# skipperro/selkies-gstreamer

Measured on AMD Instinct MI355X. Metric: encoded fps + glass-to-glass p50 ms at 1920x1080; concurrent 60fps sessions/node, higher is better.
Workload: dtype uint8 pixels / int32 integer transforms (bit-exact vs CPU reference); 1 GPU; model=H.264 Constrained Baseline CAVLC, striped stripes 64px, CRF 25, global_batch=8, seq_len=1, parallelism=session-parallel dp1 x 8 sessions/GPU, resolution=1920x1080, backend=hip, deblock=auto, me_full=True, upload_overlap=False, frames_in_flight=1, num_refs=1, numa_node_rank0=0

## Files before the change

### csrc/kernels/h264_gpu.h

```cpp
#pragma once
#include <hip/hip_runtime.h>
#include "../codec/overlay.h"
#include "../codec/h264_encoder.h"
#include "../codec/h264_frame.h"
#include "../codec/h264_deblock.h"

namespace sk {
namespace h264 {
namespace gpu {

constexpr int kMbSlotBytes = 1024;
constexpr int kSliceHdrMax = 64;
constexpr int kPackMaxSliceMbs = 16384;

struct Planes {
    uint8_t* y;
    uint8_t* u;
    uint8_t* v;
};

struct FrameArgs {
    int W, H, mb_w, mb_h, stride_y, stride_c, num_slices, rows_per_slice, fullframe;
    int full_range, me_range, me_iters;
    const uint8_t* bgrx;
// ... 6 lines not shown
    int* stripe_dirty;
    StripeState* plan_state;
    int* plan_ctl;
    const int* key_seq_host;
    int* key_dev;
    PlanConfig plan_cfg;
    SliceTask* tasks;
    MeResult* me;
    int16_t* mvfield;
    MbInfo* mbs;
    int16_t* coefs;
    uint32_t* mb_bits;
    int* mb_nbits;
    int* slice_info;
    int out_slot_bytes;
    const uint8_t* param_sets;
    const int* param_set_len;
    int param_set_stride;
    uint8_t* host_out;
    int* host_size;
    int* frame_params_dev;
    const int* frame_params_host;
    SliceTask* tasks_host;
    unsigned long long* dbg;
    const CavlcTables* cavlc_tabs;
    int num_refs;
    int deblock;
    int me_full;
    int aq_strength;
    int subpel;
    int intra4x4;
    const uint8_t* ov_img[kOverlaySlots];
    const OverlayParams* ov;
    int8_t* aq;
    DbInfo* db;
    uint4* dbe;
    int16_t* fs_mv;
    RcState* rc;
    long long* rc_slice;
    float rc_fps;
    int* rc_redo;
    int nal_per_slice;
    const int* gate;
    const uint8_t* yuv;
    int yuv_fmt;
    ltr::LtrConfig ltr_cfg;
    Planes ltr;
    size_t ltr_ny, ltr_nc;
    ltr::LtrState* ltr_state;
    ltr::LtrTask* ltr_task;
    uint32_t* ltr_part;
    uint32_t* ltr_sad;
    int* ltr_cnt;
};

#if defined(__HIPCC__)
__device__ __forceinline__ Planes ref0_planes(const FrameArgs& a, int s) {
    if (a.ltr_cfg.mode == ltr::LTR_SECOND_REF) return a.ref;
    const int j = __builtin_amdgcn_readfirstlane(a.ltr_task[s].slot);
    if (j < 0) return a.ref;
    return Planes{a.ltr.y + (size_t)j * a.ltr_ny, a.ltr.u + (size_t)j * a.ltr_nc, a.ltr.v + (size_t)j * a.ltr_nc};
}
#endif

void launch_convert_damage(const FrameArgs& a, hipStream_t s);
void launch_encode(const FrameArgs& a, hipStream_t s, bool guard = false);
void launch_frontend(const FrameArgs& a, hipStream_t s);
void launch_commit(const FrameArgs& a, hipStream_t s, bool filter = true, bool account = false);
void launch_rc_account(const FrameArgs& a, const int* sizes, int n, int stride, int per_slice, hipStream_t s);
void launch_rc_guard_sizes(const FrameArgs& a, const int* sizes, int n, int* redo, bool chained, hipStream_t s);

}
}
}
```

### csrc/kernels/h264_kernels.hip

```cpp
#include "h264_gpu.h"
#include "../codec/color.h"
#include "../codec/h264_mb.h"
#include "../codec/h264_ep.h"

namespace sk {
namespace h264 {
namespace gpu {

__device__ __forceinline__ int lane_id() { return threadIdx.x & 63; }

__device__ __forceinline__ void wave_sync() {
    __builtin_amdgcn_fence(__ATOMIC_RELEASE, "wavefront");
    __builtin_amdgcn_wave_barrier();
    __builtin_amdgcn_fence(__ATOMIC_ACQUIRE, "wavefront");
}

__device__ __forceinline__ int wave_sum(int v) {
    v += __builtin_amdgcn_mov_dpp(v, 0xB1, 0xF, 0xF, false);
    v += __builtin_amdgcn_mov_dpp(v, 0x4E, 0xF, 0xF, false);
    v += __builtin_amdgcn_mov_dpp(v, 0x124, 0xF, 0xF, false);
    v += __builtin_amdgcn_mov_dpp(v, 0x128, 0xF, 0xF, false);
    return __builtin_amdgcn_readlane(v, 0) + __builtin_amdgcn_readlane(v, 16) +
           __builtin_amdgcn_readlane(v, 32) + __builtin_amdgcn_readlane(v, 48);
}

__device__ __forceinline__ Planes ref1_planes(const FrameArgs& a, int s) {
    if (!a.ltr_cfg.slots) return a.ref1;
    const size_t j = (size_t)sk_max(a.ltr_task[s].slot, 0);
    return Planes{a.ltr.y + j * a.ltr_ny, a.ltr.u + j * a.ltr_nc, a.ltr.v + j * a.ltr_nc};
}

__device__ __forceinline__ bool split_i(const FrameArgs& a, const SliceTask& t) {
    return a.nal_per_slice > 1 && intra_split(t, a.mb_w, a.deblock, a.intra4x4);
}
__device__ __forceinline__ int slice_nals(const FrameArgs& a, const SliceTask& t) {
    if (t.final_action == ACT_NONE) return 0;
    return split_i(a, t) ? intra_sub_count(t.num_rows * a.mb_w) : 1;
}

__device__ __forceinline__ int wave_incl_scan_max(int v) {
    int l = threadIdx.x & 63;
#pragma unroll
    for (int o = 1; o < 64; o <<= 1) {
        int t = __shfl_up(v, o);
        if (l >= o) v = max(v, t);
    }
    return v;
}

__device__ __forceinline__ int wave_incl_scan(int v) {
    int l = lane_id();
#pragma unroll
    for (int o = 1; o < 64; o <<= 1) {
        int t = __shfl_up(v, o);
        if (l >= o) v += t;
    }
    return v;
}

__device__ __forceinline__ void load_cavlc_tables(CavlcTables& dst, const CavlcTables* src) {
    static_assert(sizeof(CavlcTables) % 4 == 0, "dword copy");
    const uint32_t* s = reinterpret_cast<const uint32_t*>(src);
    uint32_t* d = reinterpret_cast<uint32_t*>(&dst);
    for (int i = threadIdx.x; i < (int)(sizeof(CavlcTables) / 4); i += blockDim.x) d[i] = s[i];
}

template <int NW>
// ... 1770 lines not shown
    for (;;) {
        const int bound = cbp == 0 ? 96 : quant_bound(m.q, false, S, T, dbg, kCodeStampRow);
        if (qp + 6 > cap || bound <= mb_bit_budget(false)) break;
        qp += 6;
        wave_sync();
        cbp = quant_analyse(m.wl, m.wc, qp, false, S, m.sl, m.sc, m.q, dbg, kCodeStampRow);
    }
    STAMP_S(dbg, kCodeStampRow, 4);
    MbInfo mb;
    memset(&mb, 0, sizeof(mb));
    mb.type = MB_P_16x16;
    mb.cbp = (uint8_t)cbp;
    mb.qp = (uint8_t)qp;
    int rec_l[4], rec_c[4];
    uint32_t* g32 = reinterpret_cast<uint32_t*>(a.coefs + (size_t)idx * kCoefPerMb);
    if (cbp == 0) {
#pragma unroll
        for (int j = 0; j < 4; j++) {
            rec_l[j] = m.pred_l[j];
            rec_c[j] = m.pred_c[j];
        }
        for (int i = l; i < kCoefPerMb / 2; i += 64) g32[i] = 0;
    } else {
        recon_mb_lanes(qp, false, cbp, S, m.pred_l, m.pred_c, rec_l, rec_c, m.sl, m.sc);
        STAMP_S(dbg, kCodeStampRow, 5);
        const uint32_t* s32 = reinterpret_cast<const uint32_t*>(S.coef);
        for (int i = l; i < kCoefPerMb / 2; i += 64) g32[i] = s32[i];
    }
    STAMP_S(dbg, kCodeStampRow, 6);
    const int mvx = m.mvx, mvy = m.mvy, refi = m.refi, pmx = m.pmx, pmy = m.pmy, smx = m.smx, smy = m.smy;
    uint32_t rw = (uint32_t)rec_l[0] | ((uint32_t)rec_l[1] << 8) | ((uint32_t)rec_l[2] << 16) |
                  ((uint32_t)rec_l[3] << 24);
    *reinterpret_cast<uint32_t*>(a.rec.y + (size_t)py * a.stride_y + px) = rw;
    if (l < 32) {
        uint8_t* cr = comp ? a.rec.v : a.rec.u;
        uint32_t cw = (uint32_t)rec_c[0] | ((uint32_t)rec_c[1] << 8) | ((uint32_t)rec_c[2] << 16) |
                      ((uint32_t)rec_c[3] << 24);
        *reinterpret_cast<uint32_t*>(cr + (size_t)cy0 * a.stride_c + cx0) = cw;
    }
    STAMP_S(dbg, kCodeStampRow, 7);
    if (l == 0) {
        mb.mvx = (int16_t)mvx;
        mb.mvy = (int16_t)mvy;
        mb.ref = (uint8_t)refi;
        if (mb.cbp == 0 && refi == 0 && mvx == smx && mvy == smy) {
            mb.type = MB_P_SKIP;
        } else {
            mb.mvdx = (int16_t)(mvx - pmx);
            mb.mvdy = (int16_t)(mvy - pmy);
        }
        if (mb.cbp)
            for (int i = 0; i < 24; i++) mb.nnz[i] = S.nnz[i];
        a.mbs[idx] = mb;
    }
    STAMP_S(dbg, kCodeStampRow, 8);
}

__device__ __forceinline__ void intra_modes_wave(const int* src_l, const int* src_c, const uint8_t* topp, const uint8_t* leftp,
                                 int tl, const uint8_t* const* ctop, const uint8_t* const* cleft, const int* ctl,
                                 bool aT, bool aL, int* cdcp, int* luma_mode, int* chroma_mode,
                                 int* luma_sad = nullptr) {
    const int l = lane_id();
    const int b = l >> 2, r = l & 3;
    const int cl = l & 31, comp = cl >> 4, cb = (cl >> 2) & 3;
    const int lx = blk_x(b) * 4, ly = blk_y(b) * 4 + r;
    int dc = i16_dc(topp, leftp, aT, aL);
    int pa = 0, pb = 0, pc = 0;
    if (aT && aL) i16_plane_params(topp, leftp, tl, &pa, &pb, &pc);
    const int order[4] = {2, 0, 1, 3};
    int best_mode = 2, best_sad = 0x7fffffff;
    for (int oi = 0; oi < 4; oi++) {
        int m = order[oi];
        if ((m == 0 && !aT) || (m == 1 && !aL) || (m == 3 && !(aT && aL))) continue;
        int sad = 0;
#pragma unroll
        for (int j = 0; j < 4; j++)
            sad += sk_abs(src_l[j] - i16_pred_pixel(m, lx + j, ly, topp, leftp, tl, aT, aL, dc, pa, pb, pc));
        sad = wave_sum(sad);
        if (sad < best_sad) { best_sad = sad; best_mode = m; }
    }
    const uint8_t* ct = ctop[comp];
    const uint8_t* cf = cleft[comp];
    const int clx = (cb & 1) * 4, cly = (cb >> 1) * 4 + r;
    int qa = 0, qb = 0, qc = 0;
    if (aT && aL) chroma_plane_params(ct, cf, ctl[comp], &qa, &qb, &qc);
    if (l < 8) cdcp[l] = chroma_dc_block(l & 1, (l >> 1) & 1, ctop[l >> 2], cleft[l >> 2], aT, aL);
    wave_sync();
    const int cdc_mine = cdcp[comp * 4 + cb];
    int best_cm = 0, best_csad = 0x7fffffff;
    for (int m = 0; m < 4; m++) {
        if ((m == 1 && !aL) || (m == 2 && !aT) || (m == 3 && !(aT && aL))) continue;
        int sad = 0;
#pragma unroll
        for (int j = 0; j < 4; j++) {
            int x = clx + j, y = cly, v;
            if (m == 0) v = cdc_mine;
            else if (m == 1) v = cf[y];
            else if (m == 2) v = ct[x];
            else v = sk_clip255((qa + qb * (x - 3) + qc * (y - 3) + 16) >> 5);
            sad += sk_abs(src_c[j] - v);
        }
        sad = wave_sum(l < 32 ? sad : 0);
        if (sad < best_csad) { best_csad = sad; best_cm = m; }
    }
    *luma_mode = best_mode;
    *chroma_mode = best_cm;
// ... 139 lines not shown
            sad = quad_sum(sad);
            if (r == 0) sads[q * 9 + m] = i4_mode_ok(m, ref.hasT, ref.hasL) ? sad : -1;
        }
        wave_sync();
        const int lam = i4_lambda(t.qp);
        int total = 0;
        uint64_t modes = 0;
        for (int b = 0; b < 16; b++) {
            const int bx = blk_x(b), by = blk_y(b);
            const int ma = bx > 0 ? (int)((modes >> (4 * blk_from_xy(bx - 1, by))) & 15) : (aL ? 2 : -1);
            const int mt = by > 0 ? (int)((modes >> (4 * blk_from_xy(bx, by - 1))) & 15) : (aT ? 2 : -1);
            const int pm = i4_predicted(ma, mt);
            int best = 0x7fffffff, bm = I4_DC;
            for (int m = 0; m < 9; m++) {
                const int sd = sads[b * 9 + m];
                if (sd < 0) continue;
                const int cost = sd + lam * (m == pm ? 1 : 4);
                if (cost < best) { best = cost; bm = m; }
            }
            modes |= (uint64_t)bm << (4 * b);
            total += best;
        }
        cand.i4lo = (uint32_t)modes;
        cand.i4hi = (uint32_t)(modes >> 32);
        i4 = i4_wins(total, sad16, t.qp);
        wave_sync();
    }
    MbInfo mb;
    memset(&mb, 0, sizeof(mb));
    int qp;
    if (i4) {
        mb.type = MB_I4x4;
        mb.chroma_mode = (uint8_t)cmode;
        mb.i4lo = cand.i4lo;
        mb.i4hi = cand.i4hi;
        int rec_l[4], rec_c[4];
        qp = code_mb_i4(src_smp, src_l, src_c, pred_c, start >= 0 ? start : t.qp, t.qp, aT, aL, aTR, S, mb, rec_l,
                        rec_c, nullptr, T);
    } else {
        int rec_l[4], rec_c[4];
        qp = code_mb(src_l, pred_l, src_c, pred_c, t.qp, true, S, mb, rec_l, rec_c, nullptr, T, nullptr, 0, start,
                     true);
    }
    if (l == 0) {
        MbInfo o;
        memset(&o, 0, sizeof(o));
        o.type = i4 ? MB_I4x4 : MB_I16x16;
        o.i16_mode = (uint8_t)mode;
        o.chroma_mode = (uint8_t)cmode;
        o.qp = (uint8_t)qp;
        o.i4lo = cand.i4lo;
        o.i4hi = cand.i4hi;
        a.mbs[idx] = o;
    }
}

__global__ __launch_bounds__(256) void k_code_inter(FrameArgs a) {
    if (a.gate && *a.gate == 0) return;
    __shared__ MbScratch Sw[4];
    __shared__ QpelLds Qw[4];
    __shared__ CavlcTables T;
    const int w = threadIdx.x >> 6;
    const int nmb = a.mb_w * a.mb_h;
    const int idx = xcd_remap(blockIdx.x, gridDim.x) * 4 + w;
    const bool valid = idx < nmb;
    const int mbx = valid ? idx % a.mb_w : 0, mby = valid ? idx / a.mb_w : 0;
    const int s = mby / a.rows_per_slice;
    const SliceTask t = a.tasks[s];
    if (valid && t.final_action == ACT_SKIPALL && lane_id() == 0) {
        MbInfo z;
        memset(&z, 0, sizeof(z));
        a.mbs[idx] = z;
        a.me[idx].mvx = 0;
        a.me[idx].mvy = 0;
        a.me[idx].ref = 0;
        a.me[idx].fx = a.me[idx].fy = 0;
    }
    const bool is_p = valid && t.final_action == ACT_P, is_i = valid && t.final_action == ACT_I;
    constexpr int kTabWords = (int)(sizeof(CavlcTables) / 4);
    static_assert(kTabWords <= 512, "two dwords per thread");
    const uint32_t* tab_src = reinterpret_cast<const uint32_t*>(a.cavlc_tabs);
    const uint32_t tab0 = tab_src[threadIdx.x];
    const uint32_t tab1 = threadIdx.x + 256 < kTabWords ? tab_src[threadIdx.x + 256] : 0u;
    InterMb m;
    bool need_tables = is_i;
    if (is_p) need_tables = code_inter_begin(a, t, s, idx, mbx, mby, Sw[w], Qw[w], m) != 0;
    if (__syncthreads_or(need_tables)) {
        uint32_t* tab_dst = reinterpret_cast<uint32_t*>(&T);
        tab_dst[threadIdx.x] = tab0;
        if (threadIdx.x + 256 < kTabWords) tab_dst[threadIdx.x + 256] = tab1;
        __syncthreads();
    }
    static_assert(sizeof(QpelLds) >= 64, "the pre-pass keeps its neighbour samples in the wave's QpelLds");
    if (is_p) code_inter_finish(a, t, idx, mbx, mby, Sw[w], T, m);
    else if (is_i) intra_prep_wave(a, t, idx, mbx, mby, Sw[w], reinterpret_cast<uint8_t*>(&Qw[w]), T);
}

constexpr int kMaxRows = 16;
struct IntraEdges {
    uint8_t bot_y[kMaxRows][4][16];
    uint8_t bot_c[kMaxRows][4][2][8];
    uint8_t right_y[kMaxRows][16];
    uint8_t right_c[kMaxRows][2][8];
};

struct IntraSrc {
    uint32_t y[64];
    uint32_t c[32];
    int mode, cmode, qp, i4;
    uint32_t i4m[2];
};
constexpr int kIntraRing = 4;

template <int MAXROWS>
__global__ __launch_bounds__(64 * (MAXROWS + 1)) void k_code_intra(FrameArgs a) {
    if (a.gate && *a.gate == 0) return;
    __shared__ MbScratch Sw[MAXROWS];
    __shared__ IntraEdges E;
    __shared__ IntraSrc R[MAXROWS][kIntraRing];
    __shared__ uint8_t zero16[16];
    __shared__ CavlcTables T;
    int s = blockIdx.x;
    const SliceTask t = a.tasks[s];
    if (t.final_action != ACT_I || split_i(a, t)) return;
#ifdef SK_STAMPS
// ... 87 lines not shown
                const bool is_i4 = __builtin_amdgcn_readfirstlane(in.i4) != 0;
                int pred_l[4], pred_c[4];
                intra_pred_lanes(is_i4 ? 2 : mode, cmode, nb, tl, ctl, aT, aL, pred_l, pred_c);
                STAMP(step, 2);
                MbInfo mb;
                memset(&mb, 0, sizeof(mb));
                mb.chroma_mode = (uint8_t)cmode;
                int rec_l[4], rec_c[4];
                if (is_i4) {
                    const bool aTR = aT && mbx + 1 < a.mb_w;
                    if (l < 4) S.nbtr[l] = aTR ? E.bot_y[w - 1][(mbx + 1) & 3][l] : 0;
                    const uint32_t m0 = __builtin_amdgcn_readfirstlane(in.i4m[0]);
                    const uint32_t m1 = __builtin_amdgcn_readfirstlane(in.i4m[1]);
                    mb.i4lo = m0;
                    mb.i4hi = m1;
                    mb.type = MB_I4x4;
                    wave_sync();
                    auto smp = [&](int x, int y) __attribute__((always_inline)) -> int {
                        if (y >= 0 && x >= 0) return S.ry[y * 16 + x];
                        if (y < 0) return x < 0 ? tl : (x < 16 ? (int)nb[x] : (int)S.nbtr[x - 16]);
                        return nb[16 + y];
                    };
                    code_mb_i4(smp, src_l, src_c, pred_c, start_qp, t.qp, aT, aL, aTR, S, mb, rec_l, rec_c,
                               a.coefs + (size_t)idx * kCoefPerMb, T);
                } else {
                    mb.type = MB_I16x16;
                    mb.i16_mode = (uint8_t)mode;
                    code_mb(src_l, pred_l, src_c, pred_c, t.qp, true, S, mb, rec_l, rec_c,
                            a.coefs + (size_t)idx * kCoefPerMb, T, a.dbg, step, start_qp);
                }
                STAMP(step, 6);
                wave_sync();
                if (ly == 15)
                    for (int j = 0; j < 4; j++) E.bot_y[w][mbx & 3][lx + j] = (uint8_t)rec_l[j];
                if (lx + 3 == 15) E.right_y[w][ly] = (uint8_t)rec_l[3];
                if (l < 32) {
                    if (cly == 7)
                        for (int j = 0; j < 4; j++) E.bot_c[w][mbx & 3][comp][clx + j] = (uint8_t)rec_c[j];
                    if (clx + 3 == 7) E.right_c[w][comp][cly] = (uint8_t)rec_c[3];
                }
                const int px = mbx * 16 + lx, py = mby * 16 + ly;
                uint32_t rw = (uint32_t)rec_l[0] | ((uint32_t)rec_l[1] << 8) | ((uint32_t)rec_l[2] << 16) |
                              ((uint32_t)rec_l[3] << 24);
                *reinterpret_cast<uint32_t*>(a.rec.y + (size_t)py * a.stride_y + px) = rw;
                if (l < 32) {
                    uint8_t* crp = comp ? a.rec.v : a.rec.u;
                    uint32_t cw = (uint32_t)rec_c[0] | ((uint32_t)rec_c[1] << 8) | ((uint32_t)rec_c[2] << 16) |
                                  ((uint32_t)rec_c[3] << 24);
                    *reinterpret_cast<uint32_t*>(crp + (size_t)(mby * 8 + cly) * a.stride_c + mbx * 8 + clx) = cw;
                }
                if (l == 0) {
                    for (int i = 0; i < 24; i++) mb.nnz[i] = S.nnz[i];
                    a.mbs[idx] = mb;
                    a.me[idx].mvx = 0;
                    a.me[idx].mvy = 0;
                    a.me[idx].ref = 0;
                    a.me[idx].fx = a.me[idx].fy = 0;
                }
                STAMP(step, 7);
            }
        }
        __syncthreads();
        if (w == 0) STAMP(step, 8);
    }
#ifdef SK_STAMPS
    if (a.dbg && threadIdx.x == 0 && blockIdx.x < 32) {
        a.dbg[1024 + 2 * blockIdx.x] = t_start;
        a.dbg[1024 + 2 * blockIdx.x + 1] = __builtin_amdgcn_s_memrealtime();
        if (blockIdx.x < 32) a.dbg[1024 + 64 + 2 * blockIdx.x] = __builtin_amdgcn_s_memtime() - c_start;
        if (blockIdx.x == SK_STAMP_BLOCK) {
            a.dbg[1024 + 200] = c_start;
            a.dbg[1024 + 201] = __builtin_amdgcn_s_memtime();
            a.dbg[1024 + 202] = c_loop;
            a.dbg[1024 + 203] = steps;
        }
        if (blockIdx.x < 32) a.dbg[1024 + 64 + 2 * blockIdx.x + 1] = __builtin_amdgcn_s_getreg((31 << 11) | 4);
    }
#endif
}

__global__ __launch_bounds__(256) void k_code_intra_sub(FrameArgs a) {
    if (a.gate && *a.gate == 0) return;
    __shared__ MbScratch Sw[4];
    __shared__ uint8_t right_y[4][16];
    __shared__ uint8_t right_c[4][2][8];
    __shared__ CavlcTables T;
    const int w = threadIdx.x >> 6, l = lane_id();
    const int gw = blockIdx.x * 4 + w;
    const int s = gw / a.nal_per_slice, j = gw % a.nal_per_slice;
    bool mine = false;
    SliceTask t;
    if (s < a.num_slices) {
        t = a.tasks[s];
        mine = split_i(a, t) && j < intra_sub_count(t.num_rows * a.mb_w);
    }
    if (!__syncthreads_or(mine)) return;
    load_cavlc_tables(T, a.cavlc_tabs);
    __syncthreads();
    if (!mine) return;
    MbScratch& S = Sw[w];
    const int b = l >> 2, r = l & 3;
    const int cl = l & 31, comp = cl >> 4, cb = (cl >> 2) & 3;
    const int lx = blk_x(b) * 4, ly = blk_y(b) * 4 + r;
    const int clx = (cb & 1) * 4, cly = (cb >> 1) * 4 + r;
    const int first = t.first_row * a.mb_w;
    const int k0 = j * kIntraSubMbs, k1 = sk_min(t.num_rows * a.mb_w, k0 + kIntraSubMbs);
// ... 19 lines not shown
        const uint32_t m1 = (uint32_t)__builtin_amdgcn_readfirstlane((int)pre.i4hi);
        int src_l[4], src_c[4];
#pragma unroll
        for (int q = 0; q < 4; q++) {
            src_l[q] = (sw >> (8 * q)) & 255;
            src_c[q] = (csw >> (8 * q)) & 255;
        }
        if (k + 1 < k1) fetch(k + 1, sw, csw, pre);
        uint8_t* nb = S.nb;
        {
            int v = 0;
            if (l >= 16 && l < 32) v = aL ? right_y[w][l - 16] : 0;
            else if (l >= 48) v = aL ? right_c[w][(l >> 3) & 1][l & 7] : 0;
            nb[l] = (uint8_t)v;
        }
        wave_sync();
        int pred_l[4], pred_c[4];
        intra_pred_lanes(is_i4 ? 2 : mode, cmode, nb, 0, zc, false, aL, pred_l, pred_c);
        MbInfo mb;
        memset(&mb, 0, sizeof(mb));
        mb.chroma_mode = (uint8_t)cmode;
        int rec_l[4], rec_c[4];
        if (is_i4) {
            mb.type = MB_I4x4;
            mb.i4lo = m0;
            mb.i4hi = m1;
            auto smp = [&](int x, int y) __attribute__((always_inline)) -> int {
                if (y >= 0 && x >= 0) return S.ry[y * 16 + x];
                if (y < 0) return 0;
                return nb[16 + y];
            };
            code_mb_i4(smp, src_l, src_c, pred_c, start_qp, t.qp, false, aL, false, S, mb, rec_l, rec_c,
                       a.coefs + (size_t)idx * kCoefPerMb, T);
        } else {
            mb.type = MB_I16x16;
            mb.i16_mode = (uint8_t)mode;
            code_mb(src_l, pred_l, src_c, pred_c, t.qp, true, S, mb, rec_l, rec_c, a.coefs + (size_t)idx * kCoefPerMb,
                    T, nullptr, 0, start_qp);
        }
        wave_sync();
        if (lx + 3 == 15) right_y[w][ly] = (uint8_t)rec_l[3];
        if (l < 32 && clx + 3 == 7) right_c[w][comp][cly] = (uint8_t)rec_c[3];
        const int px = mbx * 16 + lx, py = mby * 16 + ly;
        *reinterpret_cast<uint32_t*>(a.rec.y + (size_t)py * a.stride_y + px) =
            (uint32_t)rec_l[0] | ((uint32_t)rec_l[1] << 8) | ((uint32_t)rec_l[2] << 16) | ((uint32_t)rec_l[3] << 24);
        if (l < 32) {
            uint8_t* crp = comp ? a.rec.v : a.rec.u;
            *reinterpret_cast<uint32_t*>(crp + (size_t)(mby * 8 + cly) * a.stride_c + mbx * 8 + clx) =
                (uint32_t)rec_c[0] | ((uint32_t)rec_c[1] << 8) | ((uint32_t)rec_c[2] << 16) | ((uint32_t)rec_c[3] << 24);
        }
        if (l == 0) {
            for (int i = 0; i < 24; i++) mb.nnz[i] = S.nnz[i];
            a.mbs[idx] = mb;
            a.me[idx].mvx = 0;
            a.me[idx].mvy = 0;
            a.me[idx].ref = 0;
            a.me[idx].fx = a.me[idx].fy = 0;
        }
        wave_sync();
    }
}

constexpr int kCavlcStageWords = 24;
__global__ __launch_bounds__(256) void k_cavlc(FrameArgs a) {
    if (a.gate && *a.gate == 0) return;
    __shared__ uint32_t bits_w[4][kMbSlotBytes / 4];
    __shared__ uint32_t stage_w[4][27 * kCavlcStageWords];
    __shared__ int16_t coef_w[4][kCoefPerMb];
    __shared__ MbInfo mb_w[4];
    __shared__ CavlcTables T;
    load_cavlc_tables(T, a.cavlc_tabs);
    __syncthreads();
    uint32_t* bits = bits_w[threadIdx.x >> 6];
    int16_t* coef = coef_w[threadIdx.x >> 6];
    int nmb = a.mb_w * a.mb_h;
    int idx = xcd_remap(blockIdx.x, gridDim.x) * 4 + (threadIdx.x >> 6);
    if (idx >= nmb) return;
    int mbx = idx % a.mb_w, mby = idx / a.mb_w;
    int s = mby / a.rows_per_slice;
    const SliceTask t = a.tasks[s];
    if (t.final_action != ACT_P && t.final_action != ACT_I) return;
    int l = lane_id();
    MbInfo& mb = mb_w[threadIdx.x >> 6];
    if (l < (int)(sizeof(MbInfo) / 4))
        reinterpret_cast<uint32_t*>(&mb)[l] = reinterpret_cast<const uint32_t*>(a.mbs + idx)[l];
    wave_sync();
    if (mb.type == MB_P_SKIP) {
        if (l == 0) a.mb_nbits[idx] = 0;
        return;
    }
    bool p_slice = t.final_action == ACT_P;
    int first = t.first_row * a.mb_w;
    if (split_i(a, t)) first += ((idx - first) / kIntraSubMbs) * kIntraSubMbs;
    int run = 0;
    if (p_slice) {
        int j = idx - 1;
        while (j >= first) {
            int base = j - 63;
            int m = base + l;
            bool coded = m >= first && a.mbs[m].type != MB_P_SKIP;
            unsigned long long msk = __ballot(coded);
            if (msk) {
                int hi = 63 - __clzll(msk);
                run += j - (base + hi);
                break;
            }
            run += j - sk_max(base, first) + 1;
            j = base - 1;
        }
    }
    int qp_prev = t.qp;
    {
        int j = idx - 1;
        while (j >= first) {
            int base = j - 63;
            int m = base + l;
            bool has = m >= first && mb_has_qp_delta(a.mbs[m]);
            unsigned long long msk = __ballot(has);
            if (msk) {
                int hi = 63 - __clzll(msk);
                qp_prev = a.mbs[base + hi].qp;
                break;
            }
            j = base - 1;
        }
    }
    for (int i = l; i < kMbSlotBytes / 4; i += 64) bits[i] = 0;
    uint32_t* stage_all = stage_w[threadIdx.x >> 6];
    for (int i = l; i < 27 * kCavlcStageWords; i += 64) stage_all[i] = 0;
    const int16_t* gc = a.coefs + (size_t)idx * kCoefPerMb;
    for (int i = l; i < kCoefPerMb / 2; i += 64)
        reinterpret_cast<uint32_t*>(coef)[i] = reinterpret_cast<const uint32_t*>(gc)[i];
    wave_sync();
    MbNeighbours nb;
    nb.left = mbx > 0 && idx - 1 >= first ? &a.mbs[idx - 1] : nullptr;
    nb.top = mby > t.first_row && idx - a.mb_w >= first ? &a.mbs[idx - a.mb_w] : nullptr;
    int hdr_bits = 0;
    if (l == 0) {
        AtomicBitWriter w{bits, 0};
        if (p_slice) put_ue(w, (uint32_t)run);
        int dq = mb_has_qp_delta(mb) ? (int)mb.qp - qp_prev : 0;
        write_mb_header(w, mb, p_slice, dq, p_slice ? t.num_refs : 1, nb);
        hdr_bits = (int)w.pos;
    }
    hdr_bits = __shfl(hdr_bits, 0);
    int cbp_l = mb.cbp & 15, cbp_c = (mb.cbp >> 4) & 3;
    bool i16 = mb.type == MB_I16x16;
    const int16_t* bc = nullptr;
    int maxn = 0, nc = 0;
    bool act = false;
    if (l == 0) {
        if (i16) { act = true; bc = coef + kCoefLumaDC; maxn = 16; nc = luma_nc(mb, nb, 0); }
    } else if (l <= 16) {
        int blk = l - 1;
        if (i16) {
            if (cbp_l) { act = true; bc = coef + kCoefLuma + blk * 16 + 1; maxn = 15; }
        } else if (cbp_l & (1 << (blk >> 2))) {
            act = true; bc = coef + kCoefLuma + blk * 16; maxn = 16;
        }
        if (act) nc = luma_nc(mb, nb, blk);
    } else if (l <= 18) {
        if (cbp_c) { act = true; bc = coef + kCoefChromaDC + (l - 17) * 4; maxn = 4; nc = -1; }
    } else if (l <= 26) {
        if (cbp_c == 2) {
            int k = l - 19, c = k >> 2, bb = k & 3;
            act = true; bc = coef + kCoefChromaAC + (c * 4 + bb) * 16 + 1; maxn = 15;
            nc = chroma_nc(mb, nb, c, bb);
        }
    }
    int nbits = 0;
    uint32_t* stage = stage_all + (l < 27 ? l : 0) * kCavlcStageWords;
    StageBitWriter sw{stage, 0, kCavlcStageWords * 32, false};
    if (act) {
        cavlc_block(sw, bc, maxn, nc, T);
        nbits = (int)sw.pos;
    }
    int incl = wave_incl_scan(nbits);
    int off = hdr_bits + incl - nbits;
    if (act) {
        if (!sw.ovf) {
            const uint32_t sh = (uint32_t)off & 31;
            uint32_t wi = (uint32_t)off >> 5;
            for (int k = 0; k < (nbits + 31) >> 5; k++, wi++) {
                const uint32_t v = stage[k];
                atomicOr(&bits[wi], v >> sh);
                const uint32_t lo = sh ? v << (32 - sh) : 0u;
                if (lo) atomicOr(&bits[wi + 1], lo);
            }
        } else {
// ... 307 lines not shown
    const int nmbs = sk_min(16, a.mb_w - mbx0);
    if (tid < nmbs) {
        const int idx = mby * a.mb_w + mbx0 + tid;
        const bool zero = fin == ACT_SKIPALL;
        a.mvfield[2 * idx] = zero ? 0 : a.me[idx].mvx;
        a.mvfield[2 * idx + 1] = zero ? 0 : a.me[idx].mvy;
    }
    auto copy = [&](const Planes& src, const Planes& dst) {
        {
            const int row = tid >> 4, v = tid & 15;
            if (v < nmbs) {
                const size_t o = (size_t)(mby * 16 + row) * a.stride_y + (mbx0 + v) * 16;
                *reinterpret_cast<uint4*>(dst.y + o) = *reinterpret_cast<const uint4*>(src.y + o);
            }
        }
        if (tid < 128) {
            const int comp = tid >> 6, row = (tid >> 3) & 7, v = tid & 7;
            if (2 * v < nmbs) {
                const size_t o = (size_t)(mby * 8 + row) * a.stride_c + (mbx0 + 2 * v) * 8;
                uint8_t* d = comp ? dst.v : dst.u;
                const uint8_t* sp = comp ? src.v : src.u;
                if (2 * v + 1 < nmbs && (a.stride_c & 15) == 0) {
                    *reinterpret_cast<uint4*>(d + o) = *reinterpret_cast<const uint4*>(sp + o);
                } else {
                    *reinterpret_cast<uint2*>(d + o) = *reinterpret_cast<const uint2*>(sp + o);
                    if (2 * v + 1 < nmbs)
                        *reinterpret_cast<uint2*>(d + o + 8) = *reinterpret_cast<const uint2*>(sp + o + 8);
                }
            }
        }
    };
    if (a.num_refs > 1) copy(a.ref, a.ref1);
    if (a.ltr_cfg.slots) {
        const int j = a.ltr_task[s].store_slot;
        if (j >= 0) copy(a.ref, Planes{a.ltr.y + (size_t)j * a.ltr_ny, a.ltr.u + (size_t)j * a.ltr_nc,
                                       a.ltr.v + (size_t)j * a.ltr_nc});
    }
    if (fin == ACT_SKIPALL || slice_deblock(a.deblock, a.tasks[s])) return;
    copy(a.rec, a.ref);
}

__global__ __launch_bounds__(256) void k_deblock_prep(FrameArgs a) {
    const int nmb = a.mb_w * a.mb_h;
    const int idx = xcd_remap(blockIdx.x, gridDim.x) * 4 + (threadIdx.x >> 6);
    if (idx >= nmb) return;
    const SliceTask t = a.tasks[(idx / a.mb_w) / a.rows_per_slice];
    if (t.final_action != ACT_P && t.final_action != ACT_I) return;
    if (!slice_deblock(a.deblock, t)) return;
    const int l = lane_id();
    int first = t.first_row * a.mb_w;
    if (split_i(a, t)) first += ((idx - first) / kIntraSubMbs) * kIntraSubMbs;
    const MbInfo mb = a.mbs[idx];
    int qpy = mb.qp;
    if (!mb_has_qp_delta(mb)) {
        qpy = t.qp;
        int j = idx - 1;
        while (j >= first) {
            const int base = j - 63, m = base + l;
            const unsigned long long msk = __ballot(m >= first && mb_has_qp_delta(a.mbs[m]));
            if (msk) {
                qpy = a.mbs[base + 63 - __clzll(msk)].qp;
                break;
            }
            j = base - 1;
        }
    }
    if (l == 0) a.db[idx] = db_info(mb, qpy);
}

__device__ __forceinline__ void unpack4(uint32_t w, int* d) {
    d[0] = w & 255;
    d[1] = (w >> 8) & 255;
    d[2] = (w >> 16) & 255;
    d[3] = w >> 24;
}
__device__ __forceinline__ uint32_t pack4(const int* d) {
    return (uint32_t)d[0] | ((uint32_t)d[1] << 8) | ((uint32_t)d[2] << 16) | ((uint32_t)d[3] << 24);
}

__device__ __forceinline__ DbInfo as_db(uint2 v) {
    DbInfo d;
    __builtin_memcpy(&d, &v, sizeof(d));
    return d;
}

__device__ __forceinline__ void lds_barrier() {
    __builtin_amdgcn_fence(__ATOMIC_RELEASE, "workgroup", "local");
    __builtin_amdgcn_s_barrier();
    __builtin_amdgcn_fence(__ATOMIC_ACQUIRE, "workgroup", "local");
}

__device__ __forceinline__ uint32_t db_pack_par(int i) {
    return (uint32_t)H264_DB_ALPHA[i] | ((uint32_t)H264_DB_BETA[i] << 8) | ((uint32_t)H264_DB_TC0[i][0] << 16) |
           ((uint32_t)H264_DB_TC0[i][1] << 21) | ((uint32_t)H264_DB_TC0[i][2] << 26);
}

__device__ __forceinline__ int adiff(int a, int b) { return (int)__builtin_amdgcn_sad_u16((uint32_t)a, (uint32_t)b, 0u); }
__device__ __forceinline__ int clip3(int x, int lo, int hi) { return min(max(x, lo), hi); }

template <bool kMbEdge>
__device__ __forceinline__ void db_filter_line(int* v, int bs, uint32_t par, bool chroma) {
    const int alpha = par & 255, beta = (par >> 8) & 31;
    const int tc0 = __builtin_amdgcn_ubfe(par, 16 + 5 * sk_clip(bs - 1, 0, 2), 5);
    const int p3 = v[0], p2 = v[1], p1 = v[2], p0 = v[3], q0 = v[4], q1 = v[5], q2 = v[6], q3 = v[7];
    const bool on = (bs != 0) & (adiff(p0, q0) < alpha) & (adiff(p1, p0) < beta) & (adiff(q1, q0) < beta);
    const bool ap = !chroma & (adiff(p2, p0) < beta), aq = !chroma & (adiff(q2, q0) < beta);
    const int tc = tc0 + (chroma ? 1 : (int)ap + (int)aq);
    const int d = clip3((((q0 - p0) * 4) + (p1 - q1) + 4) >> 3, -tc, tc);
    const int avg = (p0 + q0 + 1) >> 1;
    int np0 = sk_clip255(p0 + d), nq0 = sk_clip255(q0 - d);
    int np1 = ap ? p1 + clip3((p2 + avg - (p1 * 2)) >> 1, -tc0, tc0) : p1;
    int nq1 = aq ? q1 + clip3((q2 + avg - (q1 * 2)) >> 1, -tc0, tc0) : q1;
    int np2 = p2, nq2 = q2;
    if (kMbEdge) {
        const bool strong = bs == 4;
        const bool sm = adiff(p0, q0) < ((alpha >> 2) + 2);
        const bool ps = ap & sm, qs = aq & sm;
        const int sp0 = ps ? (p2 + 2 * p1 + 2 * p0 + 2 * q0 + q1 + 4) >> 3 : (2 * p1 + p0 + q1 + 2) >> 2;
        const int sq0 = qs ? (p1 + 2 * p0 + 2 * q0 + 2 * q1 + q2 + 4) >> 3 : (2 * q1 + q0 + p1 + 2) >> 2;
        np0 = strong ? sp0 : np0;
        nq0 = strong ? sq0 : nq0;
        np1 = strong ? (ps ? (p2 + p1 + p0 + q0 + 2) >> 2 : p1) : np1;
        nq1 = strong ? (qs ? (p0 + q0 + q1 + q2 + 2) >> 2 : q1) : nq1;
        np2 = (strong & ps) ? (2 * p3 + 3 * p2 + p1 + p0 + q0 + 4) >> 3 : p2;
        nq2 = (strong & qs) ? (2 * q3 + 3 * q2 + q1 + q0 + p0 + 4) >> 3 : q2;
    }
    v[1] = on ? np2 : p2;
    v[2] = on ? np1 : p1;
    v[3] = on ? np0 : p0;
    v[4] = on ? nq0 : q0;
    v[5] = on ? nq1 : q1;
    v[6] = on ? nq2 : q2;
}

__global__ __launch_bounds__(256) void k_deblock_edges(FrameArgs a) {
    const int nmb = a.mb_w * a.mb_h;
    const int idx = blockIdx.x * 256 + threadIdx.x;
    if (idx >= nmb) return;
    const int mbx = idx % a.mb_w, mby = idx / a.mb_w;
    const SliceTask t = a.tasks[mby / a.rows_per_slice];
    if (t.final_action != ACT_P && t.final_action != ACT_I) return;
    if (!slice_deblock(a.deblock, t)) return;
// ... 227 lines not shown
```

### csrc/runtime/h264_tail.h

```cpp
#pragma once
#include "hip_session.h"

namespace sk {
namespace hip_backend {

struct H264Tail {
    explicit H264Tail(const TailCtx& s) : s_(s) {}
    static EncoderConfig config(EncoderConfig c) { return c; }

    void alloc(gpu::FrameArgs& a) {
        const EncoderConfig& cfg = s_.cfg;
        const Geometry& g = s_.g;
        HipAllocs& mem = s_.mem;
        const int nmb = g.num_mbs(), ns = g.num_slices;
        a.aq = mem.dmalloc<int8_t>(nmb);
        a.db = mem.dmalloc<DbInfo>(nmb);
        a.dbe = mem.dmalloc<uint4>((size_t)3 * nmb);
        a.mbs = mem.dmalloc<MbInfo>(nmb);
        a.coefs = mem.dmalloc<int16_t>((size_t)nmb * kCoefPerMb);
        a.mb_bits = mem.dmalloc<uint32_t>((size_t)nmb * (gpu::kMbSlotBytes / 4));
        a.mb_nbits = mem.dmalloc<int>(nmb);
        int max_slice_mbs = g.rows_per_slice * g.mb_w;
        const bool can_split = g.mb_w > kIntraSubMbs;
        a.nal_per_slice = can_split ? max_nals_per_slice(g.rows_per_slice, g.mb_w) : 1;
        if (max_slice_mbs > gpu::kPackMaxSliceMbs)
            throw std::runtime_error("H.264: more than " + std::to_string(gpu::kPackMaxSliceMbs) +
                                     " macroblocks per slice is not supported");
        a.slice_info = mem.dmalloc<int>(4 * (size_t)ns * a.nal_per_slice);
        const size_t sub_rbsp = (size_t)kIntraSubMbs * gpu::kMbSlotBytes + 1024;
        const size_t max_rbsp = std::max((size_t)max_slice_mbs * gpu::kMbSlotBytes + 1024,
                                         can_split ? a.nal_per_slice * sub_rbsp : (size_t)0);
        size_t slot = (max_rbsp * 3 / 2 + 1024 + 63) & ~(size_t)63;
        a.out_slot_bytes = (int)slot;
        for (auto& o : out_) {
            o.data = mem.mapped<uint8_t>(slot * ns);
            o.size = mem.mapped<int>(ns);
        }
        std::vector<std::vector<uint8_t>> ps;
        if (cfg.fullframe) {
            ps.resize(1);
            build_parameter_sets(g.W, g.H, cfg.full_range, cfg.fps, ps[0], cfg.num_refs, ltr_slots_of(cfg));
        } else {
            ps.resize(ns);
            for (int s = 0; s < ns; s++)
                build_parameter_sets(g.W, g.slice_pix_h(s), cfg.full_range, cfg.fps, ps[s], cfg.num_refs,
                                     ltr_slots_of(cfg));
        }
        param_sets_ = ps;
        a.param_set_stride = 256;
        std::vector<uint8_t> flat((size_t)ns * 256, 0);
        std::vector<int> lens(ns, 0);
        for (int s = 0; s < ns; s++) {
            const std::vector<uint8_t>& v = ps[cfg.fullframe ? 0 : s];
            if (v.size() > 256) throw std::runtime_error("parameter sets too large");
            memcpy(&flat[(size_t)s * 256], v.data(), v.size());
            lens[s] = (int)v.size();
        }
        uint8_t* dps = mem.dmalloc<uint8_t>(flat.size());
        copy_now(dps, flat.data(), flat.size(), mem.stream);
        int* dlen = mem.dmalloc<int>(ns);
        copy_now(dlen, lens.data(), sizeof(int) * ns, mem.stream);
        a.param_sets = dps;
        a.param_set_len = dlen;
        CavlcTables* ct = mem.dmalloc<CavlcTables>(1);
        copy_now(ct, &host_cavlc_tables(), sizeof(CavlcTables), mem.stream);
        a.cavlc_tabs = ct;
        mbs_ = a.mbs;
        coefs_ = a.coefs;
        slot_bytes_ = slot;
    }

    static constexpr bool kAccountInCommit = true;
    void enqueue_backend(const gpu::FrameArgs& args, int parity, hipStream_t stream, bool redo) {
        gpu::FrameArgs a = args;
        a.host_out = out_[parity].data.dev;
        a.host_size = out_[parity].size.dev;
        gpu::launch_encode(a, stream, redo);
    }

    bool can_filter(int rc_mode, const int* snap) const {
        if (s_.cfg.deblock != 2) return s_.cfg.deblock != 0;
        const int qp = snap[1] > 0 ? snap[1] : s_.cfg.qp, pqp = snap[2] > 0 ? snap[2] : s_.cfg.paint_qp;
        return max_slice_qp(rc_mode, qp, pqp) >= kAutoDeblockQp;
    }

    void build_packets(const FrameSlot& f, int parity, std::vector<EncodedPacket>& out) {
        const Geometry& g = s_.g;
        const uint8_t* host_out = out_[parity].data.host;
        const int* h_out_size = out_[parity].size.host;
        const SliceTask* h_tasks = f.tasks.host;
        const int ns = g.num_slices;
        std::vector<long> offs(ns);
        for (int s = 0; s < ns; s++) offs[s] = (long)(s * slot_bytes_);
        if (s_.cfg.fullframe) {
            bool idr = s_.ctl.picture_is_idr(h_tasks);
            EncodedPacket pk;
            pk.y = 0; pk.w = g.W; pk.h = g.H; pk.key = idr;
            pk.data.resize(10);
            write_stripe_header(pk.data.data(), idr, f.frame, 0, g.W, g.H);
            if (idr) pk.data.insert(pk.data.end(), param_sets_[0].begin(), param_sets_[0].end());
            for (int s = 0; s < ns; s++) {
                const uint8_t* p = host_out + offs[s];
                pk.data.insert(pk.data.end(), p, p + h_out_size[s]);
            }
            out.push_back(std::move(pk));
            return;
        }
        for (int s = 0; s < ns; s++) {
            if (h_tasks[s].final_action == ACT_NONE || h_out_size[s] <= 0) continue;
            EncodedPacket pk;
            pk.y = g.slice_pix_y(s);
            pk.w = g.W;
            pk.h = g.slice_pix_h(s);
            pk.key = h_tasks[s].final_action == ACT_I && h_tasks[s].idr_on_intra;
            const uint8_t* p = host_out + offs[s];
            pk.data.assign(p, p + h_out_size[s]);
            out.push_back(std::move(pk));
        }
    }

    DebugEntry codec_debug(const std::string& s) const {
        const int64_t nmb = s_.g.num_mbs();
        const DebugEntry table[] = {
            {"mbs", mbs_, (int64_t)(nmb * sizeof(MbInfo))},
            {"coefs", coefs_, nmb * kCoefPerMb * 2},
        };
        return find_debug(table, s);
    }

   private:
    TailCtx s_;
    const MbInfo* mbs_ = nullptr;
    const int16_t* coefs_ = nullptr;
    size_t slot_bytes_ = 0;
    struct Out {
        Mapped<uint8_t> data;
        Mapped<int> size;
    } out_[2];
    std::vector<std::vector<uint8_t>> param_sets_;
};

}
}
```

Before: 6053 frames/s (1920x1080 H.264, all sessions, all GPUs).

## Add per-MB tag bytes for CAVLC skip-run/QP lookback and prefetch CAVLC inputs

Each MB coding kernel now writes a one-byte tag (coded flag, qp-delta flag, qp) into a compact array. The CAVLC and deblock-info kernels use a wave-wide lookback over 1024-tag windows instead of reading full MbInfo records per lane, which cuts scattered global loads. k_cavlc also issues its loads for tables, own/left/top MbInfo and coefficient levels before the gate check and a single block barrier, so memory latency overlaps and neighbour records come from LDS. The cost is an extra tag store per MB, extra LDS, and loads that run even when the kernel is gated off.

```diff
diff --git a/csrc/kernels/h264_gpu.h b/csrc/kernels/h264_gpu.h
--- a/csrc/kernels/h264_gpu.h
+++ b/csrc/kernels/h264_gpu.h
@@ -82,7 +82,15 @@
     uint32_t* ltr_part;
     uint32_t* ltr_sad;
     int* ltr_cnt;
+    uint8_t* mb_tag;
 };
+
+constexpr int kMbTagCoded = 0x80, kMbTagQpDelta = 0x40, kMbTagQp = 0x3F;
+SK_HD uint8_t mb_tag_of(const MbInfo& mb) {
+    return (uint8_t)((mb.type != MB_P_SKIP ? kMbTagCoded : 0) | (mb_has_qp_delta(mb) ? kMbTagQpDelta : 0) |
+                     (mb.qp & kMbTagQp));
+}
+constexpr size_t mb_tag_bytes(size_t num_mbs) { return (num_mbs + 15) & ~(size_t)15; }
 
 #if defined(__HIPCC__)
 __device__ __forceinline__ Planes ref0_planes(const FrameArgs& a, int s) {
diff --git a/csrc/kernels/h264_kernels.hip b/csrc/kernels/h264_kernels.hip
--- a/csrc/kernels/h264_kernels.hip
+++ b/csrc/kernels/h264_kernels.hip
@@ -13,6 +13,12 @@
     __builtin_amdgcn_fence(__ATOMIC_RELEASE, "wavefront");
     __builtin_amdgcn_wave_barrier();
     __builtin_amdgcn_fence(__ATOMIC_ACQUIRE, "wavefront");
+}
+
+__device__ __forceinline__ void lds_barrier() {
+    __builtin_amdgcn_fence(__ATOMIC_RELEASE, "workgroup", "local");
+    __builtin_amdgcn_s_barrier();
+    __builtin_amdgcn_fence(__ATOMIC_ACQUIRE, "workgroup", "local");
 }
 
 __device__ __forceinline__ int wave_sum(int v) {
@@ -1889,6 +1895,7 @@
         if (mb.cbp)
             for (int i = 0; i < 24; i++) mb.nnz[i] = S.nnz[i];
         a.mbs[idx] = mb;
+        a.mb_tag[idx] = mb_tag_of(mb);
     }
     STAMP_S(dbg, kCodeStampRow, 8);
 }
@@ -2134,6 +2141,7 @@
         o.i4lo = cand.i4lo;
         o.i4hi = cand.i4hi;
         a.mbs[idx] = o;
+        a.mb_tag[idx] = mb_tag_of(o);
     }
 }
 
@@ -2153,6 +2161,7 @@
         MbInfo z;
         memset(&z, 0, sizeof(z));
         a.mbs[idx] = z;
+        a.mb_tag[idx] = 0;
         a.me[idx].mvx = 0;
         a.me[idx].mvy = 0;
         a.me[idx].ref = 0;
@@ -2346,6 +2355,7 @@
                 if (l == 0) {
                     for (int i = 0; i < 24; i++) mb.nnz[i] = S.nnz[i];
                     a.mbs[idx] = mb;
+                    a.mb_tag[idx] = mb_tag_of(mb);
                     a.me[idx].mvx = 0;
                     a.me[idx].mvy = 0;
                     a.me[idx].ref = 0;
@@ -2471,6 +2481,7 @@
         if (l == 0) {
             for (int i = 0; i < 24; i++) mb.nnz[i] = S.nnz[i];
             a.mbs[idx] = mb;
+            a.mb_tag[idx] = mb_tag_of(mb);
             a.me[idx].mvx = 0;
             a.me[idx].mvy = 0;
             a.me[idx].ref = 0;
@@ -2480,30 +2491,94 @@
     }
 }
 
+__device__ __forceinline__ int tag_window_base(int end) { return ((end - 1) & ~15) - 1008; }
+__device__ __forceinline__ uint4 tag_window_load(const uint8_t* tags, int end) {
+    return *reinterpret_cast<const uint4*>(tags + sk_max(tag_window_base(end) + 16 * lane_id(), 0));
+}
+__device__ __forceinline__ uint32_t tag_bits(const uint4& v, int bit) {
+    auto nib = [bit](uint32_t w) { return (((w >> bit) & 0x01010101u) * 0x01020408u) >> 24; };
+    return nib(v.x) | (nib(v.y) << 4) | (nib(v.z) << 8) | (nib(v.w) << 12);
+}
+struct TagBack {
+    int run;
+    int qp;
+};
+__device__ __forceinline__ TagBack tag_lookback(const uint8_t* tags, uint4 tg, int idx, int first, bool want_run,
+                                                int qp_none) {
+    const int l = lane_id();
+    TagBack r{idx - first, qp_none};
+    bool need_run = want_run, need_qp = true;
+    int end = idx;
+    while (end > first) {
+        const int base = tag_window_base(end), c = base + 16 * l;
+        const int lo = sk_clip(first - c, 0, 16), hi = sk_clip(end - c, 0, 16);
+        const uint32_t in_slice = ((1u << hi) - 1u) & ~((1u << lo) - 1u);
+        if (need_run) {
+            const uint32_t cm = tag_bits(tg, 7) & in_slice;
+            const unsigned long long msk = __ballot(cm != 0);
+            if (msk) {
+                const int g = 63 - __clzll(msk);
+                r.run = idx - 1 - (base + 16 * g + 31 - __clz((int)__shfl(cm, g)));
+                need_run = false;
+            }
+        }
+        if (need_qp) {
+            const uint32_t qm = tag_bits(tg, 6) & in_slice;
+            const unsigned long long msk = __ballot(qm != 0);
+            if (msk) {
+                const int k = 31 - __clz((int)(qm | 1u));
+                const uint32_t word = k < 4 ? tg.x : k < 8 ? tg.y : k < 12 ? tg.z : tg.w;
+                r.qp = __shfl((int)((word >> (8 * (k & 3))) & kMbTagQp), 63 - __clzll(msk));
+                need_qp = false;
+            }
+        }
+        end = base;
+        if (!(need_run || need_qp) || end <= first) break;
+        tg = tag_window_load(tags, end);
+    }
+    return r;
+}
+
 constexpr int kCavlcStageWords = 24;
 __global__ __launch_bounds__(256) void k_cavlc(FrameArgs a) {
-    if (a.gate && *a.gate == 0) return;
     __shared__ uint32_t bits_w[4][kMbSlotBytes / 4];
     __shared__ uint32_t stage_w[4][27 * kCavlcStageWords];
-    __shared__ int16_t coef_w[4][kCoefPerMb];
-    __shared__ MbInfo mb_w[4];
+    __shared__ __attribute__((aligned(16))) int16_t coef_w[4][kCoefPerMb];
+    __shared__ MbInfo mb_w[4][3];
     __shared__ CavlcTables T;
-    load_cavlc_tables(T, a.cavlc_tabs);
-    __syncthreads();
-    uint32_t* bits = bits_w[threadIdx.x >> 6];
-    int16_t* coef = coef_w[threadIdx.x >> 6];
-    int nmb = a.mb_w * a.mb_h;
-    int idx = xcd_remap(blockIdx.x, gridDim.x) * 4 + (threadIdx.x >> 6);
-    if (idx >= nmb) return;
-    int mbx = idx % a.mb_w, mby = idx / a.mb_w;
-    int s = mby / a.rows_per_slice;
-    const SliceTask t = a.tasks[s];
+    const int wave = threadIdx.x >> 6, l = lane_id();
+    uint32_t* bits = bits_w[wave];
+    int16_t* coef = coef_w[wave];
+    const int nmb = a.mb_w * a.mb_h;
+    const int idx = xcd_remap(blockIdx.x, gridDim.x) * 4 + wave;
+    const bool valid = idx < nmb;
+    const int li = valid ? idx : nmb - 1;
+    const int mbx = li % a.mb_w, mby = li / a.mb_w;
+    constexpr int kTabWords = (int)(sizeof(CavlcTables) / 4);
+    static_assert(kTabWords >= 256 && kTabWords <= 512, "two dwords per thread");
+    const uint32_t* tab_src = reinterpret_cast<const uint32_t*>(a.cavlc_tabs);
+    const uint32_t tab0 = tab_src[threadIdx.x];
+    const uint32_t tab1 = tab_src[sk_min((int)threadIdx.x + 256, kTabWords - 1)];
+    const SliceTask t = a.tasks[mby / a.rows_per_slice];
+    constexpr int kInfoWords = (int)(sizeof(MbInfo) / 4);
+    static_assert(kInfoWords <= 16, "a record per 16 lanes");
+    const int who = l >> 4, iw = l & 15;
+    const int from = who == 1 && mbx > 0 ? li - 1 : who == 2 && mby > 0 ? li - a.mb_w : li;
+    const bool has_info = who < 3 && iw < kInfoWords;
+    const uint32_t info = reinterpret_cast<const uint32_t*>(a.mbs + from)[has_info ? iw : 0];
+    const uint4 tags = tag_window_load(a.mb_tag, li);
+    static_assert(kCoefPerMb * 2 % 16 == 0 && kCoefPerMb * 2 / 16 <= 64, "the levels: one uint4 per lane");
+    constexpr int kLevLanes = kCoefPerMb * 2 / 16;
+    const uint4 lev = reinterpret_cast<const uint4*>(a.coefs + (size_t)li * kCoefPerMb)[sk_min(l, kLevLanes - 1)];
+    if (a.gate && *a.gate == 0) return;
+    uint32_t* tab_dst = reinterpret_cast<uint32_t*>(&T);
+    tab_dst[threadIdx.x] = tab0;
+    if (threadIdx.x + 256 < kTabWords) tab_dst[threadIdx.x + 256] = tab1;
+    if (has_info) reinterpret_cast<uint32_t*>(&mb_w[wave][who])[iw] = info;
+    lds_barrier();
+    if (!valid) return;
     if (t.final_action != ACT_P && t.final_action != ACT_I) return;
-    int l = lane_id();
-    MbInfo& mb = mb_w[threadIdx.x >> 6];
-    if (l < (int)(sizeof(MbInfo) / 4))
-        reinterpret_cast<uint32_t*>(&mb)[l] = reinterpret_cast<const uint32_t*>(a.mbs + idx)[l];
-    wave_sync();
+    const MbInfo& mb = mb_w[wave][0];
     if (mb.type == MB_P_SKIP) {
         if (l == 0) a.mb_nbits[idx] = 0;
         return;
@@ -2511,49 +2586,16 @@
     bool p_slice = t.final_action == ACT_P;
     int first = t.first_row * a.mb_w;
     if (split_i(a, t)) first += ((idx - first) / kIntraSubMbs) * kIntraSubMbs;
-    int run = 0;
-    if (p_slice) {
-        int j = idx - 1;
-        while (j >= first) {
-            int base = j - 63;
-            int m = base + l;
-            bool coded = m >= first && a.mbs[m].type != MB_P_SKIP;
-            unsigned long long msk = __ballot(coded);
-            if (msk) {
-                int hi = 63 - __clzll(msk);
-                run += j - (base + hi);
-                break;
-            }
-            run += j - sk_max(base, first) + 1;
-            j = base - 1;
-        }
-    }
-    int qp_prev = t.qp;
-    {
-        int j = idx - 1;
-        while (j >= first) {
-            int base = j - 63;
-            int m = base + l;
-            bool has = m >= first && mb_has_qp_delta(a.mbs[m]);
-            unsigned long long msk = __ballot(has);
-            if (msk) {
-                int hi = 63 - __clzll(msk);
-                qp_prev = a.mbs[base + hi].qp;
-                break;
-            }
-            j = base - 1;
-        }
-    }
+    const TagBack back = tag_lookback(a.mb_tag, tags, idx, first, p_slice, t.qp);
+    const int run = back.run, qp_prev = back.qp;
     for (int i = l; i < kMbSlotBytes / 4; i += 64) bits[i] = 0;
-    uint32_t* stage_all = stage_w[threadIdx.x >> 6];
+    uint32_t* stage_all = stage_w[wave];
     for (int i = l; i < 27 * kCavlcStageWords; i += 64) stage_all[i] = 0;
-    const int16_t* gc = a.coefs + (size_t)idx * kCoefPerMb;
-    for (int i = l; i < kCoefPerMb / 2; i += 64)
-        reinterpret_cast<uint32_t*>(coef)[i] = reinterpret_cast<const uint32_t*>(gc)[i];
+    if (l < kLevLanes) reinterpret_cast<uint4*>(coef)[l] = lev;
     wave_sync();
     MbNeighbours nb;
-    nb.left = mbx > 0 && idx - 1 >= first ? &a.mbs[idx - 1] : nullptr;
-    nb.top = mby > t.first_row && idx - a.mb_w >= first ? &a.mbs[idx - a.mb_w] : nullptr;
+    nb.left = mbx > 0 && idx - 1 >= first ? &mb_w[wave][1] : nullptr;
+    nb.top = mby > t.first_row && idx - a.mb_w >= first ? &mb_w[wave][2] : nullptr;
     int hdr_bits = 0;
     if (l == 0) {
         AtomicBitWriter w{bits, 0};
@@ -2967,19 +3009,7 @@
     if (split_i(a, t)) first += ((idx - first) / kIntraSubMbs) * kIntraSubMbs;
     const MbInfo mb = a.mbs[idx];
     int qpy = mb.qp;
-    if (!mb_has_qp_delta(mb)) {
-        qpy = t.qp;
-        int j = idx - 1;
-        while (j >= first) {
-            const int base = j - 63, m = base + l;
-            const unsigned long long msk = __ballot(m >= first && mb_has_qp_delta(a.mbs[m]));
-            if (msk) {
-                qpy = a.mbs[base + 63 - __clzll(msk)].qp;
-                break;
-            }
-            j = base - 1;
-        }
-    }
+    if (!mb_has_qp_delta(mb)) qpy = tag_lookback(a.mb_tag, tag_window_load(a.mb_tag, idx), idx, first, false, t.qp).qp;
     if (l == 0) a.db[idx] = db_info(mb, qpy);
 }
 
@@ -2997,12 +3027,6 @@
     DbInfo d;
     __builtin_memcpy(&d, &v, sizeof(d));
     return d;
-}
-
-__device__ __forceinline__ void lds_barrier() {
-    __builtin_amdgcn_fence(__ATOMIC_RELEASE, "workgroup", "local");
-    __builtin_amdgcn_s_barrier();
-    __builtin_amdgcn_fence(__ATOMIC_ACQUIRE, "workgroup", "local");
 }
 
 __device__ __forceinline__ uint32_t db_pack_par(int i) {
diff --git a/csrc/runtime/h264_tail.h b/csrc/runtime/h264_tail.h
--- a/csrc/runtime/h264_tail.h
+++ b/csrc/runtime/h264_tail.h
@@ -17,6 +17,7 @@
         a.db = mem.dmalloc<DbInfo>(nmb);
         a.dbe = mem.dmalloc<uint4>((size_t)3 * nmb);
         a.mbs = mem.dmalloc<MbInfo>(nmb);
+        a.mb_tag = mem.dmalloc<uint8_t>(gpu::mb_tag_bytes(nmb));
         a.coefs = mem.dmalloc<int16_t>((size_t)nmb * kCoefPerMb);
         a.mb_bits = mem.dmalloc<uint32_t>((size_t)nmb * (gpu::kMbSlotBytes / 4));
         a.mb_nbits = mem.dmalloc<int>(nmb);
@@ -66,6 +67,7 @@
         copy_now(ct, &host_cavlc_tables(), sizeof(CavlcTables), mem.stream);
         a.cavlc_tabs = ct;
         mbs_ = a.mbs;
+        mb_tag_ = a.mb_tag;
         coefs_ = a.coefs;
         slot_bytes_ = slot;
     }
@@ -123,6 +125,7 @@
         const int64_t nmb = s_.g.num_mbs();
         const DebugEntry table[] = {
             {"mbs", mbs_, (int64_t)(nmb * sizeof(MbInfo))},
+            {"mb_tag", mb_tag_, nmb},
             {"coefs", coefs_, nmb * kCoefPerMb * 2},
         };
         return find_debug(table, s);
@@ -131,6 +134,7 @@
    private:
     TailCtx s_;
     const MbInfo* mbs_ = nullptr;
+    const uint8_t* mb_tag_ = nullptr;
     const int16_t* coefs_ = nullptr;
     size_t slot_bytes_ = 0;
     struct Out {
```

Measured after the change: 6045 frames/s (1920x1080 H.264, all sessions, all GPUs), median of 2. Within noise of the previous version (-0.1%).
